# AppleHolic/pytorch_sound

Measured on AMD Instinct MI355X. Metric: audio-sec/s STFT+mel+fwd/bwd, higher is better.
Workload: dtype bf16; 1 GPU; configs[1]: Conv1d separator (4 x ResBlock1, C=256, on 513-bin magnitude), 22.05 kHz, STFT 1024/256, 80 mel, batch 32 x 2 s per GPU, Adam, bf16 autocast; global_batch=32, parallelism=dp1, model_params=5520386

## Files before the change

### pytorch_sound_amd/csrc/psnd_conv.hip

```cpp
#include "psnd_common.h"
#include "psnd_conv_pair.h"
#include <stdlib.h>
#include <string.h>
#include <algorithm>
#include <atomic>

namespace {

typedef __attribute__((ext_vector_type(8))) short bf16x8;
typedef __attribute__((ext_vector_type(16))) float f32x16;
typedef unsigned short bf16_t;

__device__ __forceinline__ float bf2f(bf16_t v) { return __builtin_bit_cast(float, (unsigned)v << 16); }
__device__ __forceinline__ bf16_t f2bf(float f) {
    unsigned u = __builtin_bit_cast(unsigned, f);
    if ((u & 0x7fffffffu) > 0x7f800000u) return (bf16_t)((u >> 16) | 0x40);
    u += 0x7fffu + ((u >> 16) & 1u);
    return (bf16_t)(u >> 16);
}

typedef __bf16 hwbf16x2 __attribute__((ext_vector_type(2)));
typedef float f32x2_t __attribute__((ext_vector_type(2)));
__device__ __forceinline__ unsigned pack_bf16(float lo, float hi) {
    const f32x2_t v = {lo, hi};
// ... 1091 lines not shown
                f32x4 a = {0.f, 0.f, 0.f, 0.f};
                auto add_slabs = [&](auto nc) __attribute__((always_inline)) {
                    constexpr int NS = decltype(nc)::value;
                    f32x4 t[NS];
#pragma unroll
                    for (int u = 0; u < NS; ++u) t[u] = *reinterpret_cast<const f32x4 *>(src + (size_t)(u < splits ? u : splits - 1) * slab4);
#pragma unroll
                    for (int u = 0; u < NS; ++u) {
                        const f32x4 z = {0.f, 0.f, 0.f, 0.f};
                        a += u < splits ? t[u] : z;
                    }
                };
                if (splits <= 2) add_slabs(std::integral_constant<int, 2>{});
                else if (splits <= 4) add_slabs(std::integral_constant<int, 4>{});
                else if (splits <= 8) add_slabs(std::integral_constant<int, 8>{});
                else add_slabs(std::integral_constant<int, 16>{});
                float *dst = s_gw + j * pitch + 4 * c4;
                dst[0] = a.x, dst[1] = a.y, dst[2] = a.z, dst[3] = a.w;
            }
            __syncthreads();
            float ss4 = 0.f, dot4 = 0.f;
            for (int q = tid; q < n4; q += BD) {
                const f32x4 vv = *reinterpret_cast<const f32x4 *>(vrow + 4 * q);
#pragma unroll
                for (int e = 0; e < 4; ++e) {
                    const int i = 4 * q + e, ci = (int)__umulhi((unsigned)i, kmagic), j = i - ci * k;
                    ss4 = __builtin_fmaf(vv[e], vv[e], ss4);
                    dot4 = __builtin_fmaf(vv[e], s_gw[j * pitch + ci], dot4);
                }
            }
            for (int m = 32; m >= 1; m >>= 1) {
                ss4 += __shfl_xor(ss4, m, 64);
                dot4 += __shfl_xor(dot4, m, 64);
            }
            const int nw4 = BD >> 6;
            if ((tid & 63) == 0) red[tid >> 6] = ss4, red[16 + (tid >> 6)] = dot4;
            __syncthreads();
            float sst = 0.f, dott = 0.f;
            for (int w = 0; w < nw4; ++w) sst += red[w], dott += red[16 + w];
            const float inv = 1.f / __builtin_sqrtf(sst);
            const float dd = dott * inv;
            const float gs = g[co] * inv;
            for (int q = tid; q < n4; q += BD) {
                const f32x4 vv = *reinterpret_cast<const f32x4 *>(vrow + 4 * q);
                f32x4 o;
#pragma unroll
                for (int e = 0; e < 4; ++e) {
                    const int i = 4 * q + e, ci = (int)__umulhi((unsigned)i, kmagic), j = i - ci * k;
                    o[e] = gs * (s_gw[j * pitch + ci] - vv[e] * inv * dd);
                }
                *reinterpret_cast<f32x4 *>(gv + (size_t)co * n + 4 * q) = o;
            }
            if (tid == 0) gg[co] = dd;
            if (tid < 64 && gbias && gb_part) {
                float b = bsum;
                for (int m = 32; m >= 1; m >>= 1) b += __shfl_xor(b, m, 64);
                if (tid == 0) gbias[co] = b;
            }
            return;
        }
    }
    const size_t slab = (size_t)k * Cb * Ca;
    const float *vr = v + (size_t)co * n;
    float ss = 0.f, dot = 0.f;
    if constexpr (MANY) {
        int EP = 64;
        while (EP < n && EP < BD) EP <<= 1;
        const int NSG = BD / EP, e = tid & (EP - 1), sg = tid / EP;
        float *s_part = s_gw + pitch * k;
        for (int e0 = 0; e0 < n; e0 += EP) {
            const int ee = e0 + e;
            const bool ok = ee < n;
            const int j = (int)__umulhi((unsigned)ee, cmagic), c = ee - j * Cin;
            const float *src = gw_part + ((size_t)j * Cb + co) * Ca + c;
            float acc = 0.f;
            for (int sp0 = sg; sp0 < splits; sp0 += 8 * NSG) {
                float t[8];
#pragma unroll
                for (int u = 0; u < 8; ++u) t[u] = (ok && sp0 + u * NSG < splits) ? src[(size_t)(sp0 + u * NSG) * slab] : 0.f;
                acc += ((t[0] + t[1]) + (t[2] + t[3])) + ((t[4] + t[5]) + (t[6] + t[7]));
            }
            if (NSG > 1) {
                s_part[sg * EP + e] = acc;
                __syncthreads();
                if (sg == 0 && ok) {
                    float a2 = 0.f;
                    for (int q = 0; q < NSG; ++q) a2 += s_part[q * EP + e];
                    s_gw[j * pitch + c] = a2;
                }
                __syncthreads();
            } else if (ok) {
                s_gw[j * pitch + c] = acc;
            }
        }
    } else
    for (int e0 = tid; e0 < n; e0 += 4 * BD) {
        int jj[4], cc[4];
        float gsum[4] = {0.f, 0.f, 0.f, 0.f};
#pragma unroll
        for (int q = 0; q < 4; ++q) {
            const int e = e0 + BD * q;
            jj[q] = (int)__umulhi((unsigned)e, cmagic);
            cc[q] = e - jj[q] * Cin;
        }
        {
            float t[4][16];
#pragma unroll
            for (int q = 0; q < 4; ++q) {
                const float *src = gw_part + ((size_t)jj[q] * Cb + co) * Ca + cc[q];
#pragma unroll
                for (int u = 0; u < 16; ++u) t[q][u] = (e0 + BD * q < n && u < splits) ? src[(size_t)u * slab] : 0.f;
            }
#pragma unroll
            for (int q = 0; q < 4; ++q)
                gsum[q] += ((t[q][0] + t[q][1]) + (t[q][2] + t[q][3])) + ((t[q][4] + t[q][5]) + (t[q][6] + t[q][7])) +
                           (((t[q][8] + t[q][9]) + (t[q][10] + t[q][11])) + ((t[q][12] + t[q][13]) + (t[q][14] + t[q][15])));
        }
#pragma unroll
        for (int q = 0; q < 4; ++q)
            if (e0 + BD * q < n) s_gw[jj[q] * pitch + cc[q]] = gsum[q];
    }
    __syncthreads();
    for (int i = tid; i < n; i += BD) {
        const int ci = (int)__umulhi((unsigned)i, kmagic), j = i - ci * k;
        const float vv = vr[i];
        ss += vv * vv;
        dot += vv * s_gw[j * pitch + ci];
    }
    for (int m = 32; m >= 1; m >>= 1) {
        ss += __shfl_xor(ss, m, 64);
        dot += __shfl_xor(dot, m, 64);
    }
    const int nw = BD >> 6;
    if ((tid & 63) == 0) red[tid >> 6] = ss, red[16 + (tid >> 6)] = dot;
    __syncthreads();
    float sst = 0.f, dott = 0.f;
    for (int w = 0; w < nw; ++w) sst += red[w], dott += red[16 + w];
    const float inv = 1.f / __builtin_sqrtf(sst);
    const float d = dott * inv;
    const float gs = g[co] * inv;
    for (int i = tid; i < n; i += BD) {
        const int ci = (int)__umulhi((unsigned)i, kmagic), j = i - ci * k;
        gv[(size_t)co * n + i] = gs * (s_gw[j * pitch + ci] - vr[i] * inv * d);
    }
    if (tid == 0) gg[co] = d;
    if (tid < 64 && gbias && gb_part) {
        float b = 0.f;
        for (int sp = tid; sp < splits; sp += 64) b += gb_part[(size_t)sp * Cb + co];
        for (int m = 32; m >= 1; m >>= 1) b += __shfl_xor(b, m, 64);
        if (tid == 0) gbias[co] = b;
    }
}

template <bool MANY>
__global__ __launch_bounds__(1024) void conv_finish_kernel(const float *gw_part, const float *gb_part, int splits, const float *v,
                                                           const float *g, int Cout, int Cin, int k, int Cb, int Ca, float *gv,
                                                           float *gg, float *gbias, unsigned kmagic, unsigned cmagic) {
    extern __shared__ float s_gw[];
    __shared__ float red[32];
    conv_finish_body<MANY>(gw_part, gb_part, splits, v, g, Cin, k, Cb, Ca, gv, gg, gbias, kmagic, cmagic, blockIdx.x, s_gw, red);
}

struct FinishArgs {
    psnd_wnorm_desc d[PSND_WNORM_MAX];
    unsigned kmagic[PSND_WNORM_MAX], cmagic[PSND_WNORM_MAX];
    int blk0[PSND_WNORM_MAX + 1];
    int n;
};
template <bool MANY>
__global__ __launch_bounds__(1024) void conv_finish_multi_kernel(FinishArgs a) {
    extern __shared__ float s_gw[];
    __shared__ float red[32];
    int i = 0;
    while (i + 1 < a.n && (int)blockIdx.x >= a.blk0[i + 1]) ++i;
    const psnd_wnorm_desc &d = a.d[i];
    conv_finish_body<MANY>(d.gw_part, d.gbias_part, d.splits, d.v, d.g, d.Cin, d.k, d.Cb, d.Ca, d.gv, d.gg, d.gbias, a.kmagic[i],
                           a.cmagic[i], (int)blockIdx.x - a.blk0[i], s_gw, red);
}

}

static std::atomic<long long> g_conv_stats[4];
std::atomic<long long> g_conv_pair_stats[4];
extern "C" int psnd_conv_pair_stats(int64_t *out4, int reset) {
    if (out4)
        for (int i = 0; i < 4; ++i) out4[i] = g_conv_pair_stats[i].load();
    if (reset)
        for (int i = 0; i < 4; ++i) g_conv_pair_stats[i].store(0);
    return PSND_OK;
}
extern "C" int psnd_conv_stats(int64_t *out4, int reset) {
    if (out4)
        for (int i = 0; i < 4; ++i) out4[i] = g_conv_stats[i].load();
    if (reset)
        for (int i = 0; i < 4; ++i) g_conv_stats[i].store(0);
    return PSND_OK;
}

static int conv_row_tiles(int64_t R, int Cb, bool with3 = false) {
    const char *fe = PSND_ENV("PSND_CONV_MT");
    const int force = fe ? atoi(fe) : 0;
    if (force == 1 || force == 2) return force;
    if (PSND_ENV("PSND_CONV_MT_V1")) return ((R + 63) / 64) * ((Cb + BN - 1) / BN) >= 1024 ? 2 : 1;
    const int64_t coltiles = (Cb + BN - 1) / BN;
    int best = 1;
    int64_t best_cost = 0;
    for (int mt = 1; mt <= (with3 ? 3 : 2); ++mt) {
        const int64_t tiles = (R + 64 * mt - 1) / (64 * mt) * coltiles;
        const int64_t cost = (tiles + 511) / 512 * (100 + 64 * mt);
        if (mt == 1 || cost < best_cost) best = mt, best_cost = cost;
    }
    return best;
}

static int conv_launch(ConvParams &p, hipStream_t st, const char *what) {
    const bool combine = p.A2 != nullptr;
    const int k = p.k, Cb = p.Cb, hm = p.hm;
    if (hm > 40 || (hm > 25 && k > 7)) PSND_FAIL(PSND_E_UNSUPPORTED, "%s: tap reach %d beyond the staged A tile (25; 40 for k <= 7)", what, hm);
    const char *e3 = PSND_ENV("PSND_CONV_MT3");
    const bool can3 = !combine && p.up_role == 0 && hm <= 25 && Cb > 32 && !(e3 && atoi(e3) == 0);
    int mt = conv_row_tiles(p.R, Cb, can3);
    const bool mt3 = mt == 3;
    if (mt3) mt = 2;
    const bool narrow = Cb <= 32 && mt == 2 && p.up_role == 0 && hm <= 25 && !combine && !PSND_ENV("PSND_CONV_NO_NARROW");
    const int bm = narrow ? 256 : (mt3 ? 192 : 64 * mt), bn = narrow ? 32 : BN;
    const int kct = 32;
    size_t lds = 2 * sizeof(bf16_t) * (kct + 8) * (size_t)(bm + 2 * hm);
    if (lds < sizeof(float) * bm * (bn + 8)) lds = sizeof(float) * bm * (bn + 8);
    if (lds > 160 * 1024) PSND_FAIL(PSND_E_SHAPE, "%s: LDS %zu too large", what, lds);
    dim3 grid((unsigned)((p.R + bm - 1) / bm), (unsigned)((Cb + bn - 1) / bn));
#define PSND_CONV_LAUNCH(KT_, D_, C_, H_, U_)                                                                         \
    do {                                                                                                              \
        auto kern = mt == 2 ? conv_cl_kernel<KT_, (C_ ? 2 : (D_ > 4 ? 4 : D_)), C_, 2, 2, H_, U_> : conv_cl_kernel<KT_, D_, C_, 2, 1, H_, U_>;   \
        if constexpr (!U_ && H_ == 25 && !C_) {                                                                       \
            if (narrow && p.Ca <= 32) kern = conv_cl_kernel<KT_, 1, false, 2, 2, H_, false, 32, 1>;   \
            else if (narrow) kern = conv_cl_kernel<KT_, (D_ > 4 ? 4 : D_), false, 2, 2, H_, false, 32, 1>;            \
            else if (mt3) kern = conv_cl_kernel<KT_, (D_ > 4 ? 4 : D_), false, 2, 3, H_, false, 32, 2>;               \
        }                                                                                                             \
        if (lds > 64 * 1024) {                                                                                        \
            hipError_t e = hipFuncSetAttribute(reinterpret_cast<const void *>(kern),                                  \
                                               hipFuncAttributeMaxDynamicSharedMemorySize, (int)lds);                 \
            if (e != hipSuccess) PSND_FAIL(PSND_E_HIP, "%s: set LDS size: %s", what, hipGetErrorString(e));           \
        }                                                                                                             \
        hipLaunchKernelGGL(kern, grid, dim3(256), lds, st, p);                                                        \
    } while (0)
    if (p.up_role != 0) {
        if (k > 3 || hm > 25) PSND_FAIL(PSND_E_UNSUPPORTED, "%s: transposed-conv mode is a 2-tap convolution", what);
        if (!combine) PSND_CONV_LAUNCH(3, 8, false, 25, true);
        else PSND_CONV_LAUNCH(3, 4, true, 25, true);
    } else if (hm > 25 && !combine) PSND_CONV_LAUNCH(7, 3, false, 40, false);
    else if (hm > 25) PSND_CONV_LAUNCH(7, 3, true, 40, false);
    else if (k <= 3 && !combine) PSND_CONV_LAUNCH(3, 8, false, 25, false);
    else if (k <= 3) PSND_CONV_LAUNCH(3, 4, true, 25, false);
    else if (k <= 7 && !combine) PSND_CONV_LAUNCH(7, 3, false, 25, false);
    else if (k <= 7) PSND_CONV_LAUNCH(7, 3, true, 25, false);
    else if (k <= 11 && !combine) PSND_CONV_LAUNCH(11, 2, false, 25, false);
    else if (k <= 11) PSND_CONV_LAUNCH(11, 2, true, 25, false);
    else if (!combine) PSND_CONV_LAUNCH(16, 2, false, 25, false);
    else PSND_CONV_LAUNCH(16, 2, true, 25, false);
#undef PSND_CONV_LAUNCH
    hipError_t e_ = hipGetLastError();
    if (e_ != hipSuccess) PSND_FAIL(PSND_E_HIP, "%s: %s", what, hipGetErrorString(e_));
    g_conv_stats[mt == 2 ? 1 : 0]++;
    return PSND_OK;
}

static void conv_params_plain(ConvParams &p) {
    p.up_role = 0, p.up_u = 0, p.up_p = 0, p.up_LpO = 0, p.up_HPO = 0, p.up_LO = 0, p.up_Cr = 0;
    p.res_is_a_eff = 0;
#ifdef PSND_TRACE
    p.trace = nullptr;
#endif
}
static void wgrad_params_plain(WgradParams &p) {
    p.up_u = 0, p.up_p = 0, p.up_Lp = 0, p.up_HP = 0, p.up_LpO = 0, p.up_HPO = 0, p.up_Cr = 0;
#ifdef PSND_TRACE
    p.trace = nullptr;
#endif
}

extern "C" int psnd_conv1d_cl(const void *A, const void *A2, const void *AM, float a2_slope, const void *W, const float *bias,
                              const void *res, const void *mask_src, int64_t N, int Lp, int L, int HP, int Ca, int Cb, int k,
                              int off0, int dstep, float act_slope, float mask_slope, void *out_raw, void *out_act,
                              void *a_eff_out, void *stream) {
    if ((!A && !A2) || !W || (!out_raw && !out_act) || (A2 && !AM)) PSND_FAIL(PSND_E_ARG, "conv1d_cl: null pointer");
    if (a_eff_out && !A2) PSND_FAIL(PSND_E_ARG, "conv1d_cl: a_eff_out needs the combined operand (A2, AM)");
    if (Ca % 32 != 0 || Cb % 8 != 0) PSND_FAIL(PSND_E_SHAPE, "conv1d_cl: Ca=%d must be a multiple of 32, Cb=%d of 8", Ca, Cb);
    if (Cb % 32 != 0) PSND_FAIL(PSND_E_SHAPE, "conv1d_cl: Cb=%d must be a multiple of 32 (fragment-ordered weight pack)", Cb);
    if (k < 1 || k > 16 || N < 0 || Lp < L + 2 * HP || L <= 0) PSND_FAIL(PSND_E_SHAPE, "conv1d_cl: k=%d N=%lld Lp=%d L=%d HP=%d", k, (long long)N, Lp, L, HP);
    int hm = 0;
    for (int j = 0; j < k; ++j) {
        const int o = off0 + j * dstep;
        hm = (o < 0 ? -o : o) > hm ? (o < 0 ? -o : o) : hm;
    }
    if (hm > HP) PSND_FAIL(PSND_E_SHAPE, "conv1d_cl: tap reach %d exceeds the halo HP=%d", hm, HP);
    if (N == 0) return PSND_OK;
    if ((size_t)N * Lp * (Ca > Cb ? Ca : Cb) * 2 >= ((size_t)1 << 32) || (size_t)k * Cb * Ca * 2 >= ((size_t)1 << 32))
        PSND_FAIL(PSND_E_SHAPE, "conv1d_cl: operand larger than 4 GB (32-bit buffer offsets)");
    ConvParams p;
    conv_params_plain(p);
    p.A = static_cast<const bf16_t *>(A), p.A2 = static_cast<const bf16_t *>(A2), p.AM = static_cast<const bf16_t *>(AM);
    p.a2_slope = a2_slope;
    p.W = static_cast<const bf16_t *>(W), p.bias = bias;
    p.res = static_cast<const bf16_t *>(res), p.mask_src = static_cast<const bf16_t *>(mask_src);
    p.out_raw = static_cast<bf16_t *>(out_raw), p.out_act = static_cast<bf16_t *>(out_act);
    p.a_eff_out = static_cast<bf16_t *>(a_eff_out);
    p.R = N * (int64_t)Lp, p.Lp = Lp, p.L = L, p.HP = HP, p.Ca = Ca, p.Cb = Cb, p.k = k, p.off0 = off0, p.dstep = dstep, p.hm = hm;
    p.act_slope = act_slope, p.mask_slope = mask_slope;
#ifdef PSND_TRACE
    {
        const char *tp = PSND_ENV("PSND_TRACE_PTR");
        p.trace = tp ? reinterpret_cast<long long *>(strtoull(tp, nullptr, 0)) : nullptr;
    }
#endif
    return conv_launch(p, static_cast<hipStream_t>(stream), "conv1d_cl");
}

extern "C" int psnd_to_cl(const float *x, int64_t N, int C, int64_t T, int Lp, int HP, int Cp, int preop, void *out,
                          void *stream) {
    if (!x || !out) PSND_FAIL(PSND_E_ARG, "to_cl: null pointer");
    if (preop != 0 && preop != 1) PSND_FAIL(PSND_E_ARG, "to_cl: preop=%d (0: none, 1: log1p)", preop);
    if (Lp < T + 2 * HP || Cp < C || N > 65535 || (size_t)C * (size_t)T * 4 >= ((size_t)1 << 31) || (size_t)Lp * Cp * 2 >= ((size_t)1 << 31)) PSND_FAIL(PSND_E_SHAPE, "to_cl: Lp=%d T=%lld HP=%d Cp=%d C=%d", Lp, (long long)T, HP, Cp, C);
    if (N == 0) return PSND_OK;
    dim3 grid((Lp + 31) / 32, (Cp + 31) / 32, (unsigned)N);
    hipLaunchKernelGGL(to_cl_kernel<false>, grid, dim3(256), 0, static_cast<hipStream_t>(stream), x, static_cast<bf16_t *>(out),
                       (int)N, C, (int)T, Lp, HP, Cp, preop, nullptr, nullptr);
    PSND_CHECK_LAUNCH("to_cl");
    return PSND_OK;
// ... 288 lines not shown
        const size_t lp = (size_t)(MRW + 2 * pp.h1 + MRW + 2 * pp.h2) * (C + 8) * 2, lo = (size_t)MRW * (C + 8) * 4;
        if (lds < lp) lds = lp;
        if (lds < lo) lds = lo;
    }
    const int nwa = have_pair ? wgx * wgy * wgz : 0, nwb = have_b ? wgx * wgy * wgz : 0;
    hipLaunchKernelGGL(conv_pair_bwd_kernel, dim3((unsigned)(nwa + nwb + tiles)), dim3(256), lds, static_cast<hipStream_t>(stream), pp, wa, wb_, nwa,
                       nwb, wgx, wgy);
    PSND_CHECK_LAUNCH("conv1d_cl_pair_bwd");
    if (have_pair) g_conv_pair_stats[2]++;
    g_conv_pair_stats[3].store(splits);
    return PSND_OK;
}

extern "C" int psnd_conv1d_cl_bwd(const void *G1, const void *G2, const void *GM, float g2_slope, const void *wb, const void *xa,
                                  int64_t N, int Lp, int L, int HP, int Ca, int Cb, int k, int pad, int dil, void *gx, void *g_out,
                                  const void *gx_mask, float gx_mask_slope, const void *gx_res, float *gw_part, float *gbias_part,
                                  void *stream) {
    static const bool no_pair = PSND_ENV("PSND_NO_BWD_PAIR") != nullptr;
    if (gw_part && (k < WKT ? k - 1 : WKT - 1) * (dil < 0 ? -dil : dil) > WXR - 32)
        PSND_FAIL(PSND_E_UNSUPPORTED, "conv1d_cl_bwd: dilation %d: a tap group spans more than %d rows", dil, WXR - 32);
    int hm = 0;
    for (int j = 0; j < k; ++j) {
        const int o = pad - j * dil;
        hm = (o < 0 ? -o : o) > hm ? (o < 0 ? -o : o) : hm;
    }
    const size_t buf = sizeof(bf16_t) * 40 * (size_t)(BM + 2 * hm);
    const bool pairable = !no_pair && (G1 || G2) && (!G2 || GM) && gx && wb && xa && gw_part && k >= 1 && k <= 16 && (hm <= 25 || (hm <= 40 && k <= 7)) && hm <= HP && N > 0 &&
                          Ca % 32 == 0 && Cb % 32 == 0 && L > 0 && Lp >= L + 2 * HP &&
                          (size_t)N * Lp * (Ca > Cb ? Ca : Cb) * 2 < ((size_t)1 << 32) && (size_t)k * Cb * Ca * 2 < ((size_t)1 << 32);
    if (!pairable) {
        if (gw_part) {
            int rc = psnd_conv1d_cl_wgrad(G1, G2, GM, g2_slope, xa, N, Lp, Ca, Cb, k, -pad, dil, gw_part, gbias_part, nullptr, stream);
            if (rc != PSND_OK) return rc;
        }
        if (gx_res && gx_res == g_out) PSND_FAIL(PSND_E_UNSUPPORTED, "conv1d_cl_bwd: residual = combined gradient outside the paired launch");
        return psnd_conv1d_cl(G1, G2, GM, g2_slope, wb, nullptr, gx_res, gx_mask, N, Lp, L, HP, Cb, Ca, k, pad, -dil, 1.f, gx_mask_slope, gx,
                              nullptr, g_out, stream);
    }
    ConvParams pc;
    conv_params_plain(pc);
    pc.A = static_cast<const bf16_t *>(G1), pc.A2 = static_cast<const bf16_t *>(G2), pc.AM = static_cast<const bf16_t *>(GM);
    pc.a2_slope = g2_slope;
    pc.W = static_cast<const bf16_t *>(wb), pc.bias = nullptr;
    pc.res = static_cast<const bf16_t *>(gx_res), pc.mask_src = static_cast<const bf16_t *>(gx_mask);
    pc.out_raw = static_cast<bf16_t *>(gx), pc.out_act = nullptr, pc.a_eff_out = static_cast<bf16_t *>(g_out);
    if (gx_res && gx_res == g_out) {
        if (Ca != Cb) PSND_FAIL(PSND_E_SHAPE, "conv1d_cl_bwd: gx_res == g_out needs Ca == Cb");
        pc.res = nullptr, pc.res_is_a_eff = 1;
    }
    pc.R = N * (int64_t)Lp, pc.Lp = Lp, pc.L = L, pc.HP = HP, pc.Ca = Cb, pc.Cb = Ca, pc.k = k, pc.off0 = pad, pc.dstep = -dil, pc.hm = hm;
    pc.act_slope = 1.f, pc.mask_slope = gx_mask_slope;
    WgradParams pw;
    wgrad_params_plain(pw);
    pw.G1 = pc.A, pw.G2 = pc.A2, pw.GM = pc.AM;
    pw.xa = static_cast<const bf16_t *>(xa), pw.gw = gw_part, pw.gbias = gbias_part, pw.g_out = nullptr;
    pw.R = pc.R, pw.Ca = Ca, pw.Cb = Cb, pw.k = k, pw.off0 = -pad, pw.dstep = dil, pw.g2_slope = g2_slope;
    int64_t rps;
    const int splits = wgrad_splits(pw.R, Ca, Cb, k, &rps);
    pw.rows_per_split = (int)rps;
    const char *pe = PSND_ENV("PSND_PAIR_MT");
    const int pair_mt = pe ? atoi(pe) : 0;
    const bool can3 = !G2 && hm <= 25 && Ca > 32;
    const int mt = (pair_mt == 1 || pair_mt == 2 || (pair_mt == 3 && can3)) ? pair_mt : ((can3 && conv_row_tiles(pc.R, Ca, true) == 3) ? 3 : 2);
    const bool narrow = Ca <= 32 && mt == 2 && hm <= 25 && !G2 && (pc.R + 63) / 64 >= 1024 && !PSND_ENV("PSND_CONV_NO_NARROW");
    const int bm = narrow ? 256 : 64 * mt, bn = narrow ? 32 : BN;
    const int cgx = (int)((pc.R + bm - 1) / bm), cgy = (Ca + bn - 1) / bn;
    const bool wn = Ca <= 32 && Cb <= 32 && (pc.R + 63) / 64 >= 1024 && hm <= 25 && gw_part &&
                    ((k < 4 * WKT ? k : 4 * WKT) - 1) * (dil < 0 ? -dil : dil) <= WXRN - 32 && !PSND_ENV("PSND_CONV_NO_NARROW");
    const bool narrow1 = narrow && Cb <= 32;
    const int wk = wn ? 4 * WKT : (narrow1 ? WKT : pair_wk(k <= 3 ? 3 : (k <= 7 ? 7 : (k <= 11 ? 11 : 16)), hm > 25 ? 40 : 25));
    if (gw_part && !wn && ((k < wk ? k : wk) - 1) * (dil < 0 ? -dil : dil) > WXR - 32)
        PSND_FAIL(PSND_E_UNSUPPORTED, "conv1d_cl_bwd: dilation %d: a group of %d taps spans more than %d rows", dil, wk, WXR - 32);
    const int wgx = (Cb + 63) / 64, wgy = (Ca + 63) / 64, wgz = splits * ((k + wk - 1) / wk);
    const int nw = wgx * wgy * wgz;
    const int kct = 32;
    size_t lds = 2 * sizeof(bf16_t) * (kct + 8) * (size_t)(bm + 2 * hm);
    if (lds < sizeof(float) * bm * (bn + 8)) lds = sizeof(float) * bm * (bn + 8);
    if (lds < (size_t)kWgradLdsBytes) lds = kWgradLdsBytes;
    if (wn && lds < (size_t)kWgradNarrowLdsBytes) lds = kWgradNarrowLdsBytes;
    hipStream_t st = static_cast<hipStream_t>(stream);
#define PSND_PAIR_LAUNCH(KT_, D_, C_, H_)                                                                              \
    do {                                                                                                              \
        auto kern = mt == 2 ? conv_bwd_pair_kernel<KT_, (C_ ? 2 : (D_ > 4 ? 4 : D_)), 2, C_, 2, H_> : conv_bwd_pair_kernel<KT_, D_, 2, C_, 1, H_>;   \
        if constexpr (H_ == 25 && !C_) {                                                                              \
            if (mt == 3) kern = conv_bwd_pair_kernel<KT_, (D_ > 4 ? 4 : D_), 2, false, 3, H_>;                        \
        }                                                                                                             \
        if constexpr (H_ == 25) {                                                                                     \
            if (wn && mt == 2) kern = conv_bwd_pair_kernel<KT_, (C_ ? 2 : (D_ > 4 ? 4 : D_)), 2, C_, 2, H_, 32, 2, true>;   \
        }                                                                                                             \
        if constexpr (H_ == 25 && !C_) {                                                                              \
            if (narrow1 && wn) kern = conv_bwd_pair_kernel<KT_, 1, 2, false, 2, H_, 32, 1, true>;    \
            else if (narrow1) kern = conv_bwd_pair_kernel<KT_, 1, 2, false, 2, H_, 32, 1>;                            \
            else if (narrow) kern = conv_bwd_pair_kernel<KT_, (D_ > 4 ? 4 : D_), 2, false, 2, H_, 32, 1>;             \
        }                                                                                                             \
        if (lds > 64 * 1024) {                                                                                        \
            hipError_t e = hipFuncSetAttribute(reinterpret_cast<const void *>(kern),                                  \
                                               hipFuncAttributeMaxDynamicSharedMemorySize, (int)lds);                 \
            if (e != hipSuccess) PSND_FAIL(PSND_E_HIP, "conv1d_cl_bwd: set LDS size: %s", hipGetErrorString(e));      \
        }                                                                                                             \
        hipLaunchKernelGGL(kern, dim3((unsigned)(nw + cgx * cgy)), dim3(256), lds, st, pc, pw, nw, wgx, wgy, cgx);    \
    } while (0)
    if (hm > 25 && !G2) PSND_PAIR_LAUNCH(7, 3, false, 40);
    else if (hm > 25) PSND_PAIR_LAUNCH(7, 3, true, 40);
    else if (k <= 3 && !G2) PSND_PAIR_LAUNCH(3, 8, false, 25);
    else if (k <= 3) PSND_PAIR_LAUNCH(3, 4, true, 25);
    else if (k <= 7 && !G2) PSND_PAIR_LAUNCH(7, 3, false, 25);
    else if (k <= 7) PSND_PAIR_LAUNCH(7, 3, true, 25);
    else if (k <= 11 && !G2) PSND_PAIR_LAUNCH(11, 2, false, 25);
    else if (k <= 11) PSND_PAIR_LAUNCH(11, 2, true, 25);
    else if (!G2) PSND_PAIR_LAUNCH(16, 2, false, 25);
    else PSND_PAIR_LAUNCH(16, 2, true, 25);
#undef PSND_PAIR_LAUNCH
    PSND_CHECK_LAUNCH("conv1d_cl_bwd");
    g_conv_stats[mt == 2 ? 3 : 2]++;
    return PSND_OK;
}

extern "C" int psnd_conv1d_prep(const float *v, const float *g, const float *bias, int Cout, int Cin, int k, int Cb, int Ca,
                                void *wf, void *wb, float *bias_padded, void *stream) {
    if (!v || !g || !wf || !wb || !bias_padded) PSND_FAIL(PSND_E_ARG, "conv1d_prep: null pointer");
    if (Cb < Cout || Ca < Cin) PSND_FAIL(PSND_E_SHAPE, "conv1d_prep: padded sizes too small");
    hipStream_t s = static_cast<hipStream_t>(stream);
    const size_t nw = sizeof(bf16_t) * (size_t)k * Cb * Ca;
    hipError_t e = hipSuccess;
    if (Cb != Cout || Ca != Cin) {
        e = hipMemsetAsync(wf, 0, nw, s);
        if (e == hipSuccess) e = hipMemsetAsync(wb, 0, nw, s);
        if (e == hipSuccess) e = hipMemsetAsync(bias_padded, 0, sizeof(float) * Cb, s);
    }
    if (e != hipSuccess) PSND_FAIL(PSND_E_HIP, "conv1d_prep: memset: %s", hipGetErrorString(e));
    hipLaunchKernelGGL(conv_prep_kernel, dim3(Cout), dim3(256), 0, s, v, g, bias, Cout, Cin, k, Cb, Ca,
                       static_cast<bf16_t *>(wf), static_cast<bf16_t *>(wb), bias_padded);
    PSND_CHECK_LAUNCH("conv1d_prep");
    return PSND_OK;
}

extern "C" int psnd_conv1d_prep_multi(const void *descs_dev, int n, int total_blocks, int max_row, int which, void *stream) {
    if (!descs_dev || n <= 0 || total_blocks <= 0 || max_row <= 0 || which < 1 || which > 3) PSND_FAIL(PSND_E_ARG, "conv1d_prep_multi: bad arguments");
    const size_t lds = (size_t)PREP_ROWS * (size_t)max_row * sizeof(bf16_t);
    if (lds > 160 * 1024) PSND_FAIL(PSND_E_SHAPE, "conv1d_prep_multi: Cin * k = %d too large for the 8-row tile (use psnd_conv1d_prep)", max_row);
    if (lds > 48 * 1024) {
        hipError_t e = hipFuncSetAttribute(reinterpret_cast<const void *>(conv_prep_multi_kernel), hipFuncAttributeMaxDynamicSharedMemorySize, (int)lds);
        if (e != hipSuccess) PSND_FAIL(PSND_E_HIP, "conv1d_prep_multi: set LDS size: %s", hipGetErrorString(e));
    }
    hipLaunchKernelGGL(conv_prep_multi_kernel, dim3(total_blocks), dim3(256), lds, static_cast<hipStream_t>(stream),
                       static_cast<const PrepDesc *>(descs_dev), n, which);
    PSND_CHECK_LAUNCH("conv1d_prep_multi");
    return PSND_OK;
}

extern "C" int psnd_conv1d_wnorm_bwd(const float *gw_part, const float *gbias_part, int splits, const float *v, const float *g,
                                     int Cout, int Cin, int k, int Cb, int Ca, float *gv, float *gg, float *gbias, void *stream) {
    if (!gw_part || !v || !g || !gv || !gg || splits < 1) PSND_FAIL(PSND_E_ARG, "conv1d_wnorm_bwd: null pointer / splits");
    const size_t lds = sizeof(float) * (size_t)(Cin + 1) * k;
    if (lds > 60 * 1024) PSND_FAIL(PSND_E_SHAPE, "conv1d_wnorm_bwd: Cin*k=%d too large", Cin * k);
    const unsigned kmagic = (unsigned)((0x100000000ull + (unsigned)k - 1) / (unsigned)k);
    const unsigned cmagic = (unsigned)((0x100000000ull + (unsigned)Cin - 1) / (unsigned)Cin);
    const int threads = Cin * k >= 2048 ? 1024 : 256;
    if (splits > 16)
        hipLaunchKernelGGL(conv_finish_kernel<true>, dim3(Cout), dim3(1024), lds + 4096, static_cast<hipStream_t>(stream), gw_part,
                           gbias_part, splits, v, g, Cout, Cin, k, Cb, Ca, gv, gg, gbias, kmagic, cmagic);
    else
        hipLaunchKernelGGL(conv_finish_kernel<false>, dim3(Cout), dim3(threads), lds, static_cast<hipStream_t>(stream), gw_part,
                           gbias_part, splits, v, g, Cout, Cin, k, Cb, Ca, gv, gg, gbias, kmagic, cmagic);
    PSND_CHECK_LAUNCH("conv1d_wnorm_bwd");
    return PSND_OK;
}

extern "C" int psnd_conv1d_wnorm_bwd_multi(const psnd_wnorm_desc *descs, int n, void *stream) {
    if (!descs || n < 1 || n > PSND_WNORM_MAX) PSND_FAIL(PSND_E_ARG, "conv1d_wnorm_bwd_multi: %d descriptors (1..%d)", n, PSND_WNORM_MAX);
    FinishArgs a;
    a.n = n;
    size_t lds = 0;
    int total = 0, maxn = 0, maxsplits = 0;
    for (int i = 0; i < n; ++i) {
        const psnd_wnorm_desc &d = descs[i];
        if (!d.gw_part || !d.v || !d.g || !d.gv || !d.gg || d.splits < 1 || d.Cout < 1 || d.Cin < 1 || d.k < 1)
            PSND_FAIL(PSND_E_ARG, "conv1d_wnorm_bwd_multi: descriptor %d: null pointer / bad sizes", i);
        const size_t l = sizeof(float) * (size_t)(d.Cin + 1) * d.k;
        if (l > 60 * 1024) PSND_FAIL(PSND_E_SHAPE, "conv1d_wnorm_bwd_multi: Cin*k=%d too large", d.Cin * d.k);
        lds = l > lds ? l : lds;
        a.d[i] = d;
        a.kmagic[i] = (unsigned)((0x100000000ull + (unsigned)d.k - 1) / (unsigned)d.k);
        a.cmagic[i] = (unsigned)((0x100000000ull + (unsigned)d.Cin - 1) / (unsigned)d.Cin);
        a.blk0[i] = total;
        total += d.Cout;
        maxn = d.Cin * d.k > maxn ? d.Cin * d.k : maxn;
        maxsplits = d.splits > maxsplits ? d.splits : maxsplits;
    }
    a.blk0[n] = total;
    const int threads = maxn >= 2048 ? 1024 : 256;
    if (maxsplits > 16)
        hipLaunchKernelGGL(conv_finish_multi_kernel<true>, dim3(total), dim3(1024), lds + 4096, static_cast<hipStream_t>(stream), a);
    else
        hipLaunchKernelGGL(conv_finish_multi_kernel<false>, dim3(total), dim3(threads), lds, static_cast<hipStream_t>(stream), a);
    PSND_CHECK_LAUNCH("conv1d_wnorm_bwd_multi");
    return PSND_OK;
}

namespace {

__global__ __launch_bounds__(256) void convtr_prep_kernel(const float *v, const float *g, const float *bias, int Cin, int Cout, int K, int u,
                                                          int Cr, int Cip, bf16_t *wf, bf16_t *wb, float *bp) {
    __shared__ float red[4];
    const int ci = blockIdx.x, n = Cout * K;
    const float *vr = v + (size_t)ci * n;
    float ss = 0.f;
    for (int i = threadIdx.x; i < n; i += 256) ss += vr[i] * vr[i];
    for (int m = 32; m >= 1; m >>= 1) ss += __shfl_xor(ss, m, 64);
    if ((threadIdx.x & 63) == 0) red[threadIdx.x >> 6] = ss;
    __syncthreads();
    const float scale = g[ci] / __builtin_sqrtf(red[0] + red[1] + red[2] + red[3]);
    const int Nn = u * Cr;
    for (int i = threadIdx.x; i < n; i += 256) {
        const int co = i / K, jk = i - co * K;
        const int tap = jk / u, phi = jk - tap * u;
        const bf16_t w = f2bf(vr[i] * scale);
        wf[pack_index(2, tap, phi * Cr + co, ci, Nn, Cip)] = w;
        wb[pack_index(2, tap, ci, phi * Cr + co, Cip, Nn)] = w;
    }
    if (ci == 0)
        for (int i = threadIdx.x; i < Nn; i += 256) {
            const int co = i % Cr;
            bp[i] = (bias && co < Cout) ? bias[co] : 0.f;
        }
}

__global__ __launch_bounds__(1024) void convtr_finish_kernel(const float *gw_part, int splits, const float *v, const float *g, int Cin,
                                                             int Cout, int K, int u, int Cr, int Cip, float *gv, float *gg) {
    extern __shared__ float s_gw[];
    __shared__ float red[32];
    const int ci = blockIdx.x, n = Cout * K, Nn = u * Cr, BD = blockDim.x, tid = threadIdx.x;
    const size_t slab = (size_t)2 * Cip * Nn;
    const float *vr = v + (size_t)ci * n;
    float ss = 0.f, dot = 0.f;
    const int E = 2 * u * Cout;
    int EP = 64;
    while (EP < E && EP < BD) EP <<= 1;
    const int NSG = BD / EP, el = tid & (EP - 1), sg = tid / EP;
    float *s_part = s_gw + n;
    for (int e0 = 0; e0 < E; e0 += EP) {
        const int e = e0 + el;
        const bool ok = e < E;
        const int co = e % Cout, tp = e / Cout;
        const int tap = tp / u, phi = tp - tap * u;
        const float *src = gw_part + ((size_t)tap * Cip + ci) * Nn + phi * Cr + co;
        float a = 0.f;
        for (int sp0 = sg; sp0 < splits; sp0 += 8 * NSG) {
            float t[8];
#pragma unroll
            for (int q = 0; q < 8; ++q) t[q] = (ok && sp0 + q * NSG < splits) ? src[(size_t)(sp0 + q * NSG) * slab] : 0.f;
            a += ((t[0] + t[1]) + (t[2] + t[3])) + ((t[4] + t[5]) + (t[6] + t[7]));
        }
        if (NSG > 1) {
            s_part[sg * EP + el] = a;
            __syncthreads();
            if (sg == 0 && ok) {
                float a2 = 0.f;
                for (int q = 0; q < NSG; ++q) a2 += s_part[q * EP + el];
                s_gw[co * K + tp] = a2;
            }
            __syncthreads();
        } else if (ok) {
            s_gw[co * K + tp] = a;
        }
    }
    __syncthreads();
    for (int i = tid; i < n; i += BD) {
        const float vv = vr[i];
        ss += vv * vv;
        dot += vv * s_gw[i];
    }
    for (int m = 32; m >= 1; m >>= 1) {
        ss += __shfl_xor(ss, m, 64);
        dot += __shfl_xor(dot, m, 64);
    }
    const int nw = BD >> 6;
    if ((tid & 63) == 0) red[tid >> 6] = ss, red[16 + (tid >> 6)] = dot;
    __syncthreads();
    float sst = 0.f, dott = 0.f;
    for (int w = 0; w < nw; ++w) sst += red[w], dott += red[16 + w];
    const float inv = 1.f / __builtin_sqrtf(sst);
    const float d = dott * inv;
    const float gs = g[ci] * inv;
    for (int i = tid; i < n; i += BD) gv[(size_t)ci * n + i] = gs * (s_gw[i] - vr[i] * inv * d);
    if (tid == 0) gg[ci] = d;
}

__global__ __launch_bounds__(256) void cl_mean_act_kernel(const bf16_t *a, const bf16_t *b, const bf16_t *c, const bf16_t *d, int count,
                                                          float slope, bf16_t *out, size_t n8) {
    const size_t i = (size_t)blockIdx.x * 256 + threadIdx.x;
    if (i >= n8) return;
    const bf16_t *src[4] = {a, b, c, d};
    float acc[8] = {0.f, 0.f, 0.f, 0.f, 0.f, 0.f, 0.f, 0.f};
    for (int s = 0; s < count; ++s) {
        const uint4 q = reinterpret_cast<const uint4 *>(src[s])[i];
        const unsigned *pq = reinterpret_cast<const unsigned *>(&q);
#pragma unroll
        for (int e = 0; e < 4; ++e) acc[2 * e] += bf2f((bf16_t)(pq[e] & 0xffff)), acc[2 * e + 1] += bf2f((bf16_t)(pq[e] >> 16));
    }
    unsigned w[4];
    const float cnt = (float)count;
#pragma unroll
    for (int e = 0; e < 4; ++e) {
        const float x0 = acc[2 * e] / cnt, x1 = acc[2 * e + 1] / cnt;
        w[e] = pack_bf16(x0 > 0.f ? x0 : x0 * slope, x1 > 0.f ? x1 : x1 * slope);
    }
    reinterpret_cast<uint4 *>(out)[i] = make_uint4(w[0], w[1], w[2], w[3]);
}
struct SumGroup {
    const bf16_t *src[4];
    bf16_t *out;
    int count;
};
__global__ __launch_bounds__(256) void cl_sum2_kernel(SumGroup ga, SumGroup gb, size_t n8) {
    const size_t i = (size_t)blockIdx.x * 256 + threadIdx.x;
    if (i >= n8) return;
    const SumGroup &g = blockIdx.y == 0 ? ga : gb;
    float acc[8] = {0.f, 0.f, 0.f, 0.f, 0.f, 0.f, 0.f, 0.f};
    for (int s = 0; s < g.count; ++s) {
        const uint4 q = reinterpret_cast<const uint4 *>(g.src[s])[i];
        const unsigned *pq = reinterpret_cast<const unsigned *>(&q);
#pragma unroll
        for (int e = 0; e < 4; ++e) acc[2 * e] += bf2f((bf16_t)(pq[e] & 0xffff)), acc[2 * e + 1] += bf2f((bf16_t)(pq[e] >> 16));
    }
    unsigned w[4];
#pragma unroll
    for (int e = 0; e < 4; ++e) w[e] = pack_bf16(acc[2 * e], acc[2 * e + 1]);
    reinterpret_cast<uint4 *>(g.out)[i] = make_uint4(w[0], w[1], w[2], w[3]);
}

__global__ __launch_bounds__(256) void cl_mean_act_bwd_kernel(const bf16_t *g, const bf16_t *y, int count, float slope, bf16_t *gin, size_t n8) {
    const size_t i = (size_t)blockIdx.x * 256 + threadIdx.x;
    if (i >= n8) return;
    const uint4 qg = reinterpret_cast<const uint4 *>(g)[i], qy = reinterpret_cast<const uint4 *>(y)[i];
    const unsigned *pg = reinterpret_cast<const unsigned *>(&qg), *py = reinterpret_cast<const unsigned *>(&qy);
    unsigned w[4];
    const float cnt = (float)count;
#pragma unroll
    for (int e = 0; e < 4; ++e) {
        const float g0 = bf2f((bf16_t)(pg[e] & 0xffff)), g1 = bf2f((bf16_t)(pg[e] >> 16));
        const float y0 = bf2f((bf16_t)(py[e] & 0xffff)), y1 = bf2f((bf16_t)(py[e] >> 16));
        w[e] = pack_bf16(g0 * (y0 > 0.f ? 1.f : slope) / cnt, g1 * (y1 > 0.f ? 1.f : slope) / cnt);
    }
    reinterpret_cast<uint4 *>(gin)[i] = make_uint4(w[0], w[1], w[2], w[3]);
}

}
// ... 275 lines not shown
```

Before: 99910 audio-s/s.

## Process eight output rows per block in weight-norm backward finish kernel

Adds a row-batched path for the weight-norm gradient finish: each 256-thread block handles eight output channels, with each wave owning two rows. Split partials are loaded with 128-bit buffer loads, summed in registers and reduced with DPP/swizzle butterflies. The goal is fewer tiny blocks, better memory-level parallelism and cheaper reductions for small Cin*k layers. The cost is a larger LDS footprint, many template instantiations with higher register pressure, and a two-pass descriptor reordering in the multi launcher.

```diff
diff --git a/pytorch_sound_amd/csrc/psnd_conv.hip b/pytorch_sound_amd/csrc/psnd_conv.hip
--- a/pytorch_sound_amd/csrc/psnd_conv.hip
+++ b/pytorch_sound_amd/csrc/psnd_conv.hip
@@ -1267,28 +1267,233 @@
     }
 }
 
-template <bool MANY>
-__global__ __launch_bounds__(1024) void conv_finish_kernel(const float *gw_part, const float *gb_part, int splits, const float *v,
-                                                           const float *g, int Cout, int Cin, int k, int Cb, int Ca, float *gv,
-                                                           float *gg, float *gbias, unsigned kmagic, unsigned cmagic) {
+constexpr int FIN_ROWS = 8;
+constexpr size_t FIN_ROWS_LDS_MAX = 64 * 1024;
+__host__ __device__ inline bool conv_finish_in_rows(int Cin, int k, int Cb, int Ca, int splits) {
+    return (Cin & 3) == 0 && (Ca & 3) == 0 && splits <= 16 && Cin * k < 2048 && (splits <= 8 || Cin * k <= 1024) &&
+           sizeof(float) * FIN_ROWS * (size_t)(Cin + 1) * (size_t)k <= FIN_ROWS_LDS_MAX && (size_t)k * Cb * Ca * (size_t)splits < ((size_t)1 << 29);
+}
+
+#define FIN_WAVES(BD) ((BD) == 256 ? 4 : 1)
+
+template <int M>
+__device__ __forceinline__ float fin_lane_xor(float x) {
+    const int i = __builtin_bit_cast(int, x);
+    if constexpr (M == 1) return __builtin_bit_cast(float, __builtin_amdgcn_mov_dpp(i, 0xB1, 0xF, 0xF, true));
+    else if constexpr (M == 2) return __builtin_bit_cast(float, __builtin_amdgcn_mov_dpp(i, 0x4E, 0xF, 0xF, true));
+    else if constexpr (M == 8) return __builtin_bit_cast(float, __builtin_amdgcn_mov_dpp(i, 0x128, 0xF, 0xF, true));
+    else if constexpr (M == 4 || M == 16) return __builtin_bit_cast(float, __builtin_amdgcn_ds_swizzle(i, (M << 10) | 0x1F));
+    else return __shfl_xor(x, M, 64);
+}
+__device__ __forceinline__ float fin_butterfly(float x) {
+    x += fin_lane_xor<32>(x);
+    x += fin_lane_xor<16>(x);
+    x += fin_lane_xor<8>(x);
+    x += fin_lane_xor<4>(x);
+    x += fin_lane_xor<2>(x);
+    x += fin_lane_xor<1>(x);
+    return x;
+}
+
+template <int NS, int P>
+__device__ __forceinline__ void conv_finish_rows(const float *gw_part, const float *gb_part, int splits, const float *v, const float *g,
+                                                 int Cout, int Cin, int k, int Cb, int Ca, float *gv, float *gg, float *gbias,
+                                                 unsigned kmagic, unsigned c4magic, const int co0, float *s_gw, float *red) {
+    constexpr int RW = FIN_ROWS / 4, NU = RW * 4 * P;
+    constexpr int UB = 16 / P >= NS ? 16 / P / NS : 1;
+    static_assert(NU % UB == 0, "slab batches");
+    const int lane = threadIdx.x & 63, w = __builtin_amdgcn_readfirstlane(threadIdx.x >> 6);
+    const int n = Cin * k, n4 = n >> 2, cin4 = Cin >> 2, pitch = Cin + 1;
+    const unsigned slab_bytes = (unsigned)k * Cb * Ca * 4u;
+    const bool bias = gbias && gb_part;
+    constexpr unsigned OUTSIDE = 0x80000000u;
+    const __amdgpu_buffer_rsrc_t r_gw = make_uniform_rsrc(gw_part, (int)(slab_bytes * (unsigned)splits));
+    const __amdgpu_buffer_rsrc_t r_v = make_uniform_rsrc(v, Cout * n * 4), r_gv = make_uniform_rsrc(gv, Cout * n * 4);
+    const __amdgpu_buffer_rsrc_t r_g = make_uniform_rsrc(g, Cout * 4), r_gb = make_uniform_rsrc(gb_part, bias ? splits * Cb * 4 : 0);
+    auto unit_co = [&](int u) { return co0 + RW * w + u / (4 * P); };
+    auto unit_q0 = [&](int u) { return 64 * ((u / P) & 3) + 256 * (u % P); };
+    auto unit_live = [&](int u) { return unit_co(u) < Cout && unit_q0(u) < n4; };
+    auto fresh = [](int x) __attribute__((always_inline)) {
+        asm volatile("" : "+v"(x));
+        return x;
+    };
+    const int tap_wrap = 1 - (k - 1) * pitch;
+    auto quad_places = [&](int q, int (&at)[4]) __attribute__((always_inline)) {
+        const int ci = (int)__umulhi((unsigned)(4 * q), kmagic);
+        int j = 4 * q - ci * k;
+        at[0] = j * pitch + ci;
+#pragma unroll
+        for (int e = 1; e < 4; ++e) {
+            const bool wrap = ++j == k;
+            j = wrap ? 0 : j;
+            at[e] = at[e - 1] + (wrap ? tap_wrap : pitch);
+        }
+    };
+    auto quad_tap = [&](int q) { return cin4 == 1 ? q : (int)__umulhi((unsigned)q, c4magic); };
+    f32x4 vv[NU];
+    float bs[RW], gco[RW];
+    auto load_slabs = [&](int u, f32x4 *t) __attribute__((always_inline)) {
+        const int q = unit_q0(u) + lane;
+        const int j = quad_tap(q), c4 = q - j * cin4;
+        const unsigned off = unit_live(u) && q < n4 ? (unsigned)((j * Cb + unit_co(u)) * Ca + 4 * c4) * 4u : OUTSIDE;
+#pragma unroll
+        for (int s = 0; s < NS; ++s)
+            t[s] = __builtin_bit_cast(f32x4, __builtin_amdgcn_raw_buffer_load_b128(r_gw, (int)(s < splits ? off : OUTSIDE),
+                                                                                    (int)(slab_bytes * (unsigned)(s < splits ? s : 0)), 0));
+    };
+    auto sum_slabs = [&](int u, const f32x4 *t, int ln) __attribute__((always_inline)) {
+        const int q = unit_q0(u) + ln;
+        f32x4 a = {0.f, 0.f, 0.f, 0.f};
+#pragma unroll
+        for (int s = 0; s < NS; ++s) {
+            const f32x4 z = {0.f, 0.f, 0.f, 0.f};
+            a += s < splits ? t[s] : z;
+        }
+        if (unit_live(u) && q < n4) {
+            const int j = quad_tap(q), c4 = q - j * cin4;
+            float *dst = s_gw + (RW * w + u / (4 * P)) * (pitch * k) + j * pitch + 4 * c4;
+            dst[0] = a.x, dst[1] = a.y, dst[2] = a.z, dst[3] = a.w;
+        }
+    };
+    f32x4 t0[UB][NS];
+#pragma unroll
+    for (int u = 0; u < UB; ++u) load_slabs(u, t0[u]);
+#pragma unroll
+    for (int u = 0; u < NU; ++u) {
+        const int q = unit_q0(u) + lane;
+        vv[u] = __builtin_bit_cast(f32x4, __builtin_amdgcn_raw_buffer_load_b128(
+            r_v, (int)(unit_live(u) && q < n4 ? (unsigned)(unit_co(u) * n + 4 * q) * 4u : OUTSIDE), 0, 0));
+    }
+#pragma unroll
+    for (int rr = 0; rr < RW; ++rr) {
+        const int co = co0 + RW * w + rr;
+        gco[rr] = __builtin_bit_cast(float, __builtin_amdgcn_raw_buffer_load_b32(r_g, (int)(co < Cout ? (unsigned)co * 4u : OUTSIDE), 0, 0));
+        bs[rr] = 0.f;
+        bs[rr] += __builtin_bit_cast(float, __builtin_amdgcn_raw_buffer_load_b32(
+            r_gb, (int)(co < Cout && lane < splits ? (unsigned)(lane * Cb + co) * 4u : OUTSIDE), 0, 0));
+    }
+    {
+        const int ln = fresh(lane);
+#pragma unroll
+        for (int u = 0; u < UB; ++u) sum_slabs(u, t0[u], ln);
+    }
+#pragma unroll
+    for (int u0 = UB; u0 < NU; u0 += UB) {
+        f32x4 t[UB][NS];
+#pragma unroll
+        for (int u = 0; u < UB; ++u) load_slabs(u0 + u, t[u]);
+        const int ln = fresh(lane);
+#pragma unroll
+        for (int u = 0; u < UB; ++u) sum_slabs(u0 + u, t[u], ln);
+    }
+    __syncthreads();
+#pragma unroll
+    for (int rv = 0; rv < RW * 4; ++rv) {
+        const float *s_row = s_gw + (RW * w + rv / 4) * (pitch * k);
+        float ss4 = 0.f, dot4 = 0.f;
+        if (unit_live(rv * P)) {
+            const int ln = fresh(lane);
+#pragma unroll
+            for (int p = 0; p < P; ++p) {
+                const int q = unit_q0(rv * P + p) + ln;
+                if (q < n4) {
+                    int at[4];
+                    quad_places(q, at);
+#pragma unroll
+                    for (int e = 0; e < 4; ++e) {
+                        ss4 = __builtin_fmaf(vv[rv * P + p][e], vv[rv * P + p][e], ss4);
+                        dot4 = __builtin_fmaf(vv[rv * P + p][e], s_row[at[e]], dot4);
+                    }
+                }
+            }
+            ss4 = fin_butterfly(ss4), dot4 = fin_butterfly(dot4);
+        }
+        if (lane == 0) red[4 * RW * w + rv] = ss4, red[4 * FIN_ROWS + 4 * RW * w + rv] = dot4;
+    }
+    __syncthreads();
+#pragma unroll
+    for (int rr = 0; rr < RW; ++rr) {
+        const int co = co0 + RW * w + rr;
+        if (co >= Cout) continue;
+        const float *s_row = s_gw + (RW * w + rr) * (pitch * k);
+        float sst = 0.f, dott = 0.f;
+        for (int vw = 0; vw < 4; ++vw) sst += red[4 * (RW * w + rr) + vw], dott += red[4 * FIN_ROWS + 4 * (RW * w + rr) + vw];
+        const float inv = 1.f / __builtin_sqrtf(sst);
+        const float dd = dott * inv;
+        const float gs = gco[rr] * inv;
+#pragma unroll
+        for (int vp = 0; vp < 4 * P; ++vp) {
+            const int u = rr * 4 * P + vp, q = unit_q0(u) + fresh(lane);
+            if (unit_live(u) && q < n4) {
+                f32x4 o;
+                int at[4];
+                quad_places(q, at);
+#pragma unroll
+                for (int e = 0; e < 4; ++e) o[e] = gs * (s_row[at[e]] - vv[u][e] * inv * dd);
+                __builtin_amdgcn_raw_buffer_store_b128(__builtin_bit_cast(__attribute__((__vector_size__(4 * sizeof(unsigned)))) unsigned, o), r_gv,
+                                                       (int)((unsigned)(co * n + 4 * q) * 4u), 0, 0);
+            }
+        }
+        if (lane == 0) gg[co] = dd;
+        if (bias) {
+            const float b = fin_butterfly(bs[rr]);
+            if (lane == 0) gbias[co] = b;
+        }
+    }
+}
+
+__device__ __forceinline__ void conv_finish_rows_any(const float *gw_part, const float *gb_part, int splits, const float *v, const float *g,
+                                                     int Cout, int Cin, int k, int Cb, int Ca, float *gv, float *gg, float *gbias,
+                                                     unsigned kmagic, unsigned c4magic, const int b, float *s_gw, float *red) {
+    auto run = [&](auto ns, auto p) __attribute__((always_inline)) {
+        conv_finish_rows<decltype(ns)::value, decltype(p)::value>(gw_part, gb_part, splits, v, g, Cout, Cin, k, Cb, Ca, gv, gg, gbias, kmagic,
+                                                                  c4magic, FIN_ROWS * b, s_gw, red);
+    };
+    auto by_slots = [&](auto p) __attribute__((always_inline)) {
+        if (splits <= 2) run(std::integral_constant<int, 2>{}, p);
+        else if (splits <= 4) run(std::integral_constant<int, 4>{}, p);
+        else if (splits <= 8 || decltype(p)::value == 2) run(std::integral_constant<int, 8>{}, p);
+        else if constexpr (decltype(p)::value == 1) run(std::integral_constant<int, 16>{}, p);
+    };
+    if (Cin * k <= 1024) by_slots(std::integral_constant<int, 1>{});
+    else by_slots(std::integral_constant<int, 2>{});
+}
+
+template <bool MANY, int BD>
+__global__ __launch_bounds__(BD, FIN_WAVES(BD)) void conv_finish_kernel(const float *gw_part, const float *gb_part, int splits, const float *v,
+                                                         const float *g, int Cout, int Cin, int k, int Cb, int Ca, float *gv,
+                                                         float *gg, float *gbias, unsigned kmagic, unsigned cmagic, unsigned c4magic) {
     extern __shared__ float s_gw[];
-    __shared__ float red[32];
+    __shared__ float red[8 * FIN_ROWS];
+    if constexpr (!MANY && BD == 256) {
+        if (conv_finish_in_rows(Cin, k, Cb, Ca, splits)) {
+            conv_finish_rows_any(gw_part, gb_part, splits, v, g, Cout, Cin, k, Cb, Ca, gv, gg, gbias, kmagic, c4magic, blockIdx.x, s_gw, red);
+            return;
+        }
+    }
     conv_finish_body<MANY>(gw_part, gb_part, splits, v, g, Cin, k, Cb, Ca, gv, gg, gbias, kmagic, cmagic, blockIdx.x, s_gw, red);
 }
 
 struct FinishArgs {
     psnd_wnorm_desc d[PSND_WNORM_MAX];
-    unsigned kmagic[PSND_WNORM_MAX], cmagic[PSND_WNORM_MAX];
+    unsigned kmagic[PSND_WNORM_MAX], cmagic[PSND_WNORM_MAX], c4magic[PSND_WNORM_MAX];
     int blk0[PSND_WNORM_MAX + 1];
     int n;
 };
-template <bool MANY>
-__global__ __launch_bounds__(1024) void conv_finish_multi_kernel(FinishArgs a) {
+template <bool MANY, int BD>
+__global__ __launch_bounds__(BD, FIN_WAVES(BD)) void conv_finish_multi_kernel(FinishArgs a) {
     extern __shared__ float s_gw[];
-    __shared__ float red[32];
+    __shared__ float red[8 * FIN_ROWS];
     int i = 0;
     while (i + 1 < a.n && (int)blockIdx.x >= a.blk0[i + 1]) ++i;
     const psnd_wnorm_desc &d = a.d[i];
+    if constexpr (!MANY && BD == 256) {
+        if (conv_finish_in_rows(d.Cin, d.k, d.Cb, d.Ca, d.splits)) {
+            conv_finish_rows_any(d.gw_part, d.gbias_part, d.splits, d.v, d.g, d.Cout, d.Cin, d.k, d.Cb, d.Ca, d.gv, d.gg, d.gbias, a.kmagic[i],
+                                 a.c4magic[i], (int)blockIdx.x - a.blk0[i], s_gw, red);
+            return;
+        }
+    }
     conv_finish_body<MANY>(d.gw_part, d.gbias_part, d.splits, d.v, d.g, d.Cin, d.k, d.Cb, d.Ca, d.gv, d.gg, d.gbias, a.kmagic[i],
                            a.cmagic[i], (int)blockIdx.x - a.blk0[i], s_gw, red);
 }
@@ -1883,17 +2088,30 @@
 extern "C" int psnd_conv1d_wnorm_bwd(const float *gw_part, const float *gbias_part, int splits, const float *v, const float *g,
                                      int Cout, int Cin, int k, int Cb, int Ca, float *gv, float *gg, float *gbias, void *stream) {
     if (!gw_part || !v || !g || !gv || !gg || splits < 1) PSND_FAIL(PSND_E_ARG, "conv1d_wnorm_bwd: null pointer / splits");
-    const size_t lds = sizeof(float) * (size_t)(Cin + 1) * k;
+    size_t lds = sizeof(float) * (size_t)(Cin + 1) * k;
     if (lds > 60 * 1024) PSND_FAIL(PSND_E_SHAPE, "conv1d_wnorm_bwd: Cin*k=%d too large", Cin * k);
     const unsigned kmagic = (unsigned)((0x100000000ull + (unsigned)k - 1) / (unsigned)k);
     const unsigned cmagic = (unsigned)((0x100000000ull + (unsigned)Cin - 1) / (unsigned)Cin);
+    const unsigned cin4 = Cin >= 4 ? (unsigned)Cin >> 2 : 1u, c4magic = (unsigned)((0x100000000ull + cin4 - 1) / cin4);
     const int threads = Cin * k >= 2048 ? 1024 : 256;
     if (splits > 16)
-        hipLaunchKernelGGL(conv_finish_kernel<true>, dim3(Cout), dim3(1024), lds + 4096, static_cast<hipStream_t>(stream), gw_part,
-                           gbias_part, splits, v, g, Cout, Cin, k, Cb, Ca, gv, gg, gbias, kmagic, cmagic);
-    else
-        hipLaunchKernelGGL(conv_finish_kernel<false>, dim3(Cout), dim3(threads), lds, static_cast<hipStream_t>(stream), gw_part,
-                           gbias_part, splits, v, g, Cout, Cin, k, Cb, Ca, gv, gg, gbias, kmagic, cmagic);
+        hipLaunchKernelGGL((conv_finish_kernel<true, 1024>), dim3(Cout), dim3(1024), lds + 4096, static_cast<hipStream_t>(stream), gw_part,
+                           gbias_part, splits, v, g, Cout, Cin, k, Cb, Ca, gv, gg, gbias, kmagic, cmagic, c4magic);
+    else if (threads == 1024)
+        hipLaunchKernelGGL((conv_finish_kernel<false, 1024>), dim3(Cout), dim3(1024), lds, static_cast<hipStream_t>(stream), gw_part,
+                           gbias_part, splits, v, g, Cout, Cin, k, Cb, Ca, gv, gg, gbias, kmagic, cmagic, c4magic);
+    else {
+        const bool rows = conv_finish_in_rows(Cin, k, Cb, Ca, splits);
+        if (rows) lds *= FIN_ROWS;
+        if (lds > 48 * 1024) {
+            hipError_t e = hipFuncSetAttribute(reinterpret_cast<const void *>(conv_finish_kernel<false, 256>),
+                                               hipFuncAttributeMaxDynamicSharedMemorySize, (int)FIN_ROWS_LDS_MAX);
+            if (e != hipSuccess) PSND_FAIL(PSND_E_HIP, "conv1d_wnorm_bwd: set LDS size: %s", hipGetErrorString(e));
+        }
+        hipLaunchKernelGGL((conv_finish_kernel<false, 256>), dim3(rows ? (Cout + FIN_ROWS - 1) / FIN_ROWS : Cout), dim3(256), lds,
+                           static_cast<hipStream_t>(stream), gw_part, gbias_part, splits, v, g, Cout, Cin, k, Cb, Ca, gv, gg, gbias, kmagic,
+                           cmagic, c4magic);
+    }
     PSND_CHECK_LAUNCH("conv1d_wnorm_bwd");
     return PSND_OK;
 }
@@ -1902,8 +2120,8 @@
     if (!descs || n < 1 || n > PSND_WNORM_MAX) PSND_FAIL(PSND_E_ARG, "conv1d_wnorm_bwd_multi: %d descriptors (1..%d)", n, PSND_WNORM_MAX);
     FinishArgs a;
     a.n = n;
-    size_t lds = 0;
-    int total = 0, maxn = 0, maxsplits = 0;
+    size_t lds = 0, lds_rows = 0;
+    int maxn = 0, maxsplits = 0;
     for (int i = 0; i < n; ++i) {
         const psnd_wnorm_desc &d = descs[i];
         if (!d.gw_part || !d.v || !d.g || !d.gv || !d.gg || d.splits < 1 || d.Cout < 1 || d.Cin < 1 || d.k < 1)
@@ -1911,20 +2129,39 @@
         const size_t l = sizeof(float) * (size_t)(d.Cin + 1) * d.k;
         if (l > 60 * 1024) PSND_FAIL(PSND_E_SHAPE, "conv1d_wnorm_bwd_multi: Cin*k=%d too large", d.Cin * d.k);
         lds = l > lds ? l : lds;
-        a.d[i] = d;
-        a.kmagic[i] = (unsigned)((0x100000000ull + (unsigned)d.k - 1) / (unsigned)d.k);
-        a.cmagic[i] = (unsigned)((0x100000000ull + (unsigned)d.Cin - 1) / (unsigned)d.Cin);
-        a.blk0[i] = total;
-        total += d.Cout;
+        const size_t lr = conv_finish_in_rows(d.Cin, d.k, d.Cb, d.Ca, d.splits) ? FIN_ROWS * l : l;
+        lds_rows = lr > lds_rows ? lr : lds_rows;
         maxn = d.Cin * d.k > maxn ? d.Cin * d.k : maxn;
         maxsplits = d.splits > maxsplits ? d.splits : maxsplits;
     }
+    const bool rows = maxsplits <= 16 && maxn < 2048;
+    int total = 0, m = 0;
+    for (int pass = 0; pass < 2; ++pass)
+        for (int i = 0; i < n; ++i) {
+            const psnd_wnorm_desc &d = descs[i];
+            const bool in_rows = rows && conv_finish_in_rows(d.Cin, d.k, d.Cb, d.Ca, d.splits);
+            if (in_rows != (pass == 1)) continue;
+            a.d[m] = d;
+            a.kmagic[m] = (unsigned)((0x100000000ull + (unsigned)d.k - 1) / (unsigned)d.k);
+            a.cmagic[m] = (unsigned)((0x100000000ull + (unsigned)d.Cin - 1) / (unsigned)d.Cin);
+            const unsigned cin4 = d.Cin >= 4 ? (unsigned)d.Cin >> 2 : 1u;
+            a.c4magic[m] = (unsigned)((0x100000000ull + cin4 - 1) / cin4);
+            a.blk0[m++] = total;
+            total += in_rows ? (d.Cout + FIN_ROWS - 1) / FIN_ROWS : d.Cout;
+        }
     a.blk0[n] = total;
-    const int threads = maxn >= 2048 ? 1024 : 256;
     if (maxsplits > 16)
-        hipLaunchKernelGGL(conv_finish_multi_kernel<true>, dim3(total), dim3(1024), lds + 4096, static_cast<hipStream_t>(stream), a);
-    else
-        hipLaunchKernelGGL(conv_finish_multi_kernel<false>, dim3(total), dim3(threads), lds, static_cast<hipStream_t>(stream), a);
+        hipLaunchKernelGGL((conv_finish_multi_kernel<true, 1024>), dim3(total), dim3(1024), lds + 4096, static_cast<hipStream_t>(stream), a);
+    else if (!rows)
+        hipLaunchKernelGGL((conv_finish_multi_kernel<false, 1024>), dim3(total), dim3(1024), lds, static_cast<hipStream_t>(stream), a);
+    else {
+        if (lds_rows > 48 * 1024) {
+            hipError_t e = hipFuncSetAttribute(reinterpret_cast<const void *>(conv_finish_multi_kernel<false, 256>),
+                                               hipFuncAttributeMaxDynamicSharedMemorySize, (int)FIN_ROWS_LDS_MAX);
+            if (e != hipSuccess) PSND_FAIL(PSND_E_HIP, "conv1d_wnorm_bwd_multi: set LDS size: %s", hipGetErrorString(e));
+        }
+        hipLaunchKernelGGL((conv_finish_multi_kernel<false, 256>), dim3(total), dim3(256), lds_rows, static_cast<hipStream_t>(stream), a);
+    }
     PSND_CHECK_LAUNCH("conv1d_wnorm_bwd_multi");
     return PSND_OK;
 }
```

After: 101,200 audio-s/s, median of 6. 1.2% higher.
